# zju3dv/pvnet

Hardware: AMD Instinct MI355X
Metric: RANSAC votings/s (480x640, 9 kpts, batch 32) + HBM GB/s vs roofline (higher is better)
Workload: dtype f32 decisions (bf16x3 MFMA products, f32 accumulate; pairs inside the f32 rounding band re-evaluated in the reference's f32 order); refinement f64; 1 GPU; BASELINE.json configs[2]: batch=32 synthetic 480x640 fields per GPU, 9 keypoints, 1024 hypotheses, inlier_thresh 0.99, int64 mask, planar strided field; batch_per_gpu=32, global_batch=32, h=480, w=640, vn=9, hn=1024, mask_radius=40, field=noisy (0.05 rad + 10% outliers), N(0,1) background, input_sets_cycled=4, streams=6

## Files before the change

### include/pvnet_vote.h

```cpp
#ifndef PVNET_VOTE_H_
#define PVNET_VOTE_H_

#include <stddef.h>
#include <stdint.h>

#ifdef __cplusplus
extern "C" {
#endif

#define PVNET_VOTE_ABI_VERSION 9

#define PVNET_E_BADARG      (-1)
#define PVNET_E_WORKSPACE   (-2)
#define PVNET_E_UNSUPPORTED (-3)

#define PVNET_MASK_U8   0
#define PVNET_MASK_I16  1
#define PVNET_MASK_I32  2
#define PVNET_MASK_I64  3
#define PVNET_MASK_F32  4
#define PVNET_MASK_LOGITS_F32 5

#define PVNET_F_LITERAL   1u
#define PVNET_F_NO_REFINE 2u
// ... 87 lines not shown
                           float* out_kpts, int32_t* out_status,
                           void* workspace, size_t workspace_bytes, void* stream, float* stage_ms);

int pvnet_vote_v3_stage_repeat(const void* mask, int mask_dtype, const int64_t mask_strides[3],
                               const float* vertex, const int64_t vertex_strides[5],
                               int b, int h, int w, int vn, int hn,
                               float inlier_thresh, int min_num, int max_num,
                               uint64_t seed, int image_base, const int32_t* idxs, uint32_t flags,
                               float* out_kpts, int32_t* out_status,
                               void* workspace, size_t workspace_bytes, void* stream,
                               int stage, int repeats, float* avg_ms);

int pvnet_vote_band_margin(float thresh, uint32_t* out_stats, int b, int h, int w, int vn, int hn, int max_num,
                           void* workspace, size_t workspace_bytes, void* stream);

int pvnet_rccl_load(const char* path);
int pvnet_rccl_unique_id(void* id128);
int pvnet_rccl_comm_init(void** comm, int nranks, const void* id128, int rank);
int pvnet_rccl_comm_ranks(void* comm, int* nranks);
int pvnet_rccl_comm_destroy(void* comm);
int pvnet_vote_allgather(const float* local, float* all, size_t count_per_rank, void* comm, void* stream);

int pvnet_vote_confidence(const float* kpts, float thresh, float* out_conf, uint32_t vote_flags, int b, int h, int w,
                          int vn, int hn, int max_num, void* workspace, size_t workspace_bytes, void* stream);
int pvnet_vote_distribution(const float* mean, float* out_cov, int b, int h, int w, int vn, int hn, int max_num,
                            void* workspace, size_t workspace_bytes, void* stream);

size_t pvnet_motion_workspace_bytes(int b, int h, int w, int vn);
int pvnet_motion_voting(const void* mask, int mask_dtype, const int64_t mask_strides[3], const float* vertex,
                        const int64_t vertex_strides[5], int b, int h, int w, int vn, float* out_pts, void* workspace,
// ... 43 lines not shown
```

### pvnet_amd/_abi.py

```python
from __future__ import annotations

import ctypes as C
import functools
import os
from typing import NamedTuple

_HERE = os.path.dirname(os.path.abspath(__file__))
LIB_PATH = os.path.join(_HERE, "libpvnet_vote.so")
DEV_LIB_PATH = os.path.join(_HERE, "libpvnet_vote_dev.so")
TUNING_KNOBS = ("PVNET_SCORE_MODE", "PVNET_SCORE_WGS_PER_CU", "PVNET_SCORE_HPL", "PVNET_SCORE_CHUNK", "PVNET_COMPACT_KG",
                "PVNET_SCORE_XCD", "PVNET_SCORE_ATOMIC", "PVNET_SCORE_LDS_KB", "PVNET_SCORE_ACC", "PVNET_EXACT_FOLD",
                "PVNET_SCORE_RUNS", "PVNET_SCORE_CULL", "PVNET_CULL_Q_MILLI", "PVNET_DEV_STAGES")

ABI_VERSION = 9
E_BADARG, E_WORKSPACE, E_UNSUPPORTED = -1, -2, -3
MASK_U8, MASK_I16, MASK_I32, MASK_I64, MASK_F32, MASK_LOGITS_F32 = 0, 1, 2, 3, 4, 5
F_LITERAL = 1
F_NO_REFINE = 2
F_VERTEX_F16, F_VERTEX_BF16, F_LOGITS_F16, F_LOGITS_BF16 = 4, 8, 16, 32
F_APPROX = 64
F_BAND_STATS = 128
F_CONCURRENT = 256
F_CULL_ALL, F_CULL_NONE = 512, 1024
S_SKIPPED, S_SINGULAR, S_NO_INLIER, S_OVERFLOW = 1, 2, 4, 8
# ... 20 lines not shown
_WS_TAIL = [_int] * 6 + [_ptr, _size, _ptr]
_OP_GENERATE = [_ptr, _ptr, _ptr, _ptr, _int, _int, _int, _ptr]
_OP_VOTE = [_ptr, _ptr, _ptr, _ptr, _int, _int, _int, _f32, _ptr]
PROTOTYPES = {
    "pvnet_vote_abi_version": (_int, []),
    "pvnet_vote_build_info": (C.c_char_p, []),
    "pvnet_vote_tuning_reload": (None, []),
    "pvnet_vote_layout": (_int, [_int] * 6 + [C.POINTER(Layout)]),
    "pvnet_vote_workspace_bytes": (_size, [_int] * 6),
    "pvnet_vote_v3": (_int, _V3),
    "pvnet_vote_v3_logits": (_int, [_ptr, _i64p, _int, _ptr, _i64p] + _V3[5:]),
    "pvnet_vote_v3_prepared": (_int, _V3[3:6] + [_int] + _V3[6:]),
    "pvnet_vote_v3_profiled": (_int, _V3 + [C.POINTER(_f32)]),
    "pvnet_vote_v3_stage_repeat": (_int, _V3 + [_int, _int, C.POINTER(_f32)]),
    "pvnet_vote_band_margin": (_int, [_f32, _ptr] + _WS_TAIL),
    "pvnet_vote_confidence": (_int, [_ptr, _f32, _ptr, C.c_uint32] + _WS_TAIL),
    "pvnet_vote_distribution": (_int, [_ptr, _ptr] + _WS_TAIL),
    "pvnet_motion_workspace_bytes": (_size, [_int] * 4),
    "pvnet_motion_voting": (_int, [_ptr, _int, _i64p, _ptr, _i64p] + [_int] * 4 + [_ptr, _ptr, _size, _ptr]),
    "pvnet_motion_voting_typed": (_int, [_ptr, _int, _i64p, _ptr, _i64p] + [_int] * 4 + [C.c_uint32, _ptr, _ptr, _size, _ptr]),
    "pvnet_generate_hypothesis": (_int, _OP_GENERATE),
    "pvnet_voting_for_hypothesis": (_int, _OP_VOTE),
    "pvnet_generate_hypothesis_vanishing_point": (_int, _OP_GENERATE),
    "pvnet_voting_for_hypothesis_vanishing_point": (_int, _OP_VOTE),
    "pvnet_pose_solve": (_int, [_ptr, _int, _i64p, _ptr, _ptr, _int, _ptr] + [_int] * 4 + [_ptr] * 4),
    "pvnet_pose_metrics_workspace_bytes": (_size, [_int] * 3),
    "pvnet_pose_metrics": (_int, [_ptr, _ptr, _int] + [_ptr] * 4 + [_int, _int, _ptr, _ptr, _int, _int, _int, C.POINTER(C.c_double)] +
                           [_ptr] * 4 + [_size, _ptr]),
    "pvnet_nearest_workspace_bytes": (_size, [_int, _int]),
    "pvnet_nearest_point_idx": (_int, [_ptr, _ptr, _ptr] + [_int] * 5 + [_ptr, _size, _ptr]),
# ... 334 lines not shown
```

### pvnet_amd/csrc/epilogues.hip

```cpp
#include "vote_common.h"

namespace pvd {
namespace {

__global__ __launch_bounds__(256) void band_margin_kernel(VoteParams P, unsigned* __restrict__ out) {
    PVNET_SPARE_VGPRS(119);
    extern __shared__ __attribute__((aligned(16))) char smem[];
    uint4* s_t = reinterpret_cast<uint4*>(smem);
    float4* s_raw = reinterpret_cast<float4*>(s_t + 8 * TILE_U4);
    const int k = blockIdx.x % P.vn, bi = blockIdx.x / P.vn, grp = blockIdx.y;
    const int lane = threadIdx.x & 63, col = lane & 31, half = lane >> 5, wave = threadIdx.x >> 6;
    const int tn = P.ctrl[bi * CTRL_STRIDE + C_TN];
    if (P.ctrl[bi * CTRL_STRIDE + C_NCHUNKS] <= 0 || grp * 256 >= tn) return;
    const size_t bk = (size_t)bi * P.vn + k;
    const int tpad = (tn + PAD - 1) / PAD * PAD;
    const int32_t* const org = band_origin_ptr(P, bk);
    const float ox = (float)org[0], oy = (float)org[1];
    const float rho = band_rho(tn);
    {
        const int i = threadIdx.x, p = grp * 256 + i;
        float4 q = make_float4(0.f, 0.f, 0.f, 0.f);
        if (p < tpad) q = P.rec[bk * P.cap + p];
        s_raw[i] = q;
        uint4 r0, r1, r2, r3;
// ... 33 lines not shown
                if (!(fabsf(x) >= BAND_CLEAN)) ++nband;
                if ((x > 0.f) != lit) {
                    ++ndis;
                    worst = fmaxf(worst, fabsf(x));
                }
            }
        }
    }
    unsigned* o = out + bk * 4;
    if (worst > 0.f) atomicMax(o, __float_as_uint(worst));
    if (ndis) atomicAdd(o + 1, ndis);
    if (nband) atomicAdd(o + 2, nband);
    atomicAdd(o + 3, ntest);
}

__global__ __launch_bounds__(256) void ts_collect_kernel(const unsigned long long* __restrict__ stamps, int n,
                                                         unsigned long long* __restrict__ acc, int clear) {
    PVNET_SPARE_VGPRS(39);
    unsigned long long lo = ~0ull, hi = 0ull;
    for (int i = threadIdx.x; i < n; i += 256) {
        const unsigned long long a = stamps[2 * i], b = stamps[2 * i + 1];
        lo = a < lo ? a : lo;
        hi = b > hi ? b : hi;
    }
    __shared__ unsigned long long s_lo[256], s_hi[256];
    s_lo[threadIdx.x] = lo;
    s_hi[threadIdx.x] = hi;
    __syncthreads();
    if (threadIdx.x == 0) {
        for (int i = 1; i < 256; ++i) {
// ... 298 lines not shown
    if (!out_stats) return PVNET_E_BADARG;
    VoteParams P;
    int rc = params_for_workspace(P, b, h, w, vn, hn, max_num, workspace, workspace_bytes);
    if (rc) return rc;
    if (!(thresh >= 1e-3f && thresh < 1.f) || !P.mode) return PVNET_E_UNSUPPORTED;
    P.thresh = thresh;
    P.tau = (float)(sqrt(1.0 - (double)thresh * thresh) / (double)thresh);
    P.kband = band_constant(thresh);
    hipStream_t s = static_cast<hipStream_t>(stream);
    PV_HIP(hipMemsetAsync(out_stats, 0, sizeof(uint32_t) * 4 * (size_t)b * vn, s));
    const size_t lds = 8 * TILE_U4 * sizeof(uint4) + 256 * sizeof(float4);
    hipLaunchKernelGGL(band_margin_kernel, dim3((unsigned)(b * vn), (unsigned)((P.cap + 255) / 256)), dim3(256), lds, s, P,
                       reinterpret_cast<unsigned*>(out_stats));
    PV_LAUNCH_CHECK();
    return 0;
}

static int motion_layout(int b, int h, int w, int vn, size_t off[4], int* words, int* nseg) {
    if (b <= 0 || h <= 0 || w <= 0 || vn <= 0) return PVNET_E_BADARG;
    if ((long long)h * w > (1ll << 30) || b > 65535 || vn > 65535) return PVNET_E_UNSUPPORTED;
    *words = (int)(((long long)h * w + 63) / 64);
    *nseg = (*words + SEG_WORDS - 1) / SEG_WORDS;
    off[0] = 0;
    off[1] = align_up(off[0] + sizeof(uint64_t) * (size_t)b * *words, 256);
    off[2] = align_up(off[1] + sizeof(int32_t) * 2 * (size_t)b * *nseg, 256);
    off[3] = align_up(off[2] + sizeof(double) * 2 * (size_t)b * *nseg * vn, 256);
    return 0;
}

size_t pvnet_motion_workspace_bytes(int b, int h, int w, int vn) {
// ... 102 lines not shown
```

### pvnet_amd/csrc/k4_exact_body.h

```cpp
#pragma once
#include "vote_common.h"

namespace pvd {
namespace {

__device__ __forceinline__ void vote8x(unsigned& acc, float& dm, float a0, float b0, float a1, float b1, float a2, float b2,
                                       float a3, float b3, float a4, float b4, float a5, float b5, float a6, float b6,
                                       float a7, float b7) {
    float x0, x1, x2, x3;
    unsigned w0, w1;
    asm volatile(
        "v_sub_f32_e64 %2, %8, |%9|\n"
        "v_sub_f32_e64 %3, %10, |%11|\n"
        "v_sub_f32_e64 %4, %12, |%13|\n"
        "v_sub_f32_e64 %5, %14, |%15|\n"
        "v_min3_f32 %1, %1, |%2|, |%3|\n"
        "v_cvt_pknorm_u16_f32 %6, %2, %3\n"
        "v_sub_f32_e64 %2, %16, |%17|\n"
        "v_sub_f32_e64 %3, %18, |%19|\n"
        "v_min3_f32 %1, %1, |%4|, |%5|\n"
        "v_cvt_pknorm_u16_f32 %7, %4, %5\n"
        "v_sub_f32_e64 %4, %20, |%21|\n"
        "v_sub_f32_e64 %5, %22, |%23|\n"
        "v_add3_u32 %0, %6, %7, %0\n"
// ... 377 lines not shown
            for (int t = 0; t < MH; ++t) {
                flg[t] = dmn[t] >= BAND_CLEAN ? 0u : 1u;
                cnt[t] = flg[t] ? 0u : cnt[t];
            }
        }
        if (!RUNS) flush_counts<MH>(P.counts + it.bk * P.hn_pad + it.h0, cnt);
        list_flagged_cells<MH>(P, flg, it.h0, lane, wave, colx, halfx, s_cells, &s_ncell);
        lds_barrier();
        clk.mark(2);
        const int ncell = s_ncell;
        if (ncell > 0) {
            int tid2 = threadIdx.x;
            asm volatile("" : "+v"(tid2));
            const int grp = tid2 >> 4, q = tid2 & 15;
            int ntests = 0;
            for (int e = grp; e < ncell; e += 16) {
                const unsigned cell = s_cells[e];
                const int hl = (int)(cell & 1023u), hf = (int)((cell >> 10) & 1u);
                unsigned m = cell >> 11;
                const float2 hv = s_hyp[hl];
                const int row = (q >> 2) * 8 + hf * 4 + (q & 3);
                int votes = 0;
                while (m) {
                    const int g = __ffs((int)m) - 1;
                    m &= m - 1u;
                    const int t0 = FOLD ? nti - 1 - g : 0, t1 = FOLD ? t0 + 1 : nti;
                    for (int tile = t0; tile < t1; ++tile) {
                        const float4 r = s_raw[tile * 32 + row];
                        votes += inlier_literal(r.x, r.y, r.z, r.w, hv.x, hv.y, P.thresh) ? 1 : 0;
                        ++ntests;
                    }
                }
                add_cell_votes(P.counts + it.bk * P.hn_pad + it.hslice + hl, votes, q);
            }
            add_band_stats(P, tid2, q, ncell, ntests);
        }
    }
    if (RUNS && run_key >= 0) flush_counts<MH>(P.counts + run_bk * P.hn_pad + run_h0, cnt);
    if (!HEAD) clk.finish(P);
}
#undef PV_XS
#undef PV_LO
#undef PV_HI

}
// ... 2 lines not shown
```

### pvnet_amd/csrc/k4_score_cull.hip

```cpp
#include "vote_common.h"
#include "k4_exact_body.h"

namespace pvd {
namespace {

template <bool TIMED, bool TAIL, bool WIDE>
__device__ __forceinline__ void score_cull_body(VoteParams P) {
    constexpr int MH = 8;
    if (WIDE) PVNET_SPARE_VGPRS(135); else PVNET_SPARE_VGPRS(127);
    if (!TAIL) PhaseClock<TIMED>::stamp(P, 0);
    extern __shared__ __attribute__((aligned(16))) char smem[];
    int tx0 = threadIdx.x;
    if (TAIL) asm volatile("" : "+v"(tx0));
    const int lane = tx0 & 63, col = lane & 31, half = lane >> 5;
    const int wave = __builtin_amdgcn_readfirstlane((int)(threadIdx.x >> 6));
    uint4* s_t = reinterpret_cast<uint4*>(smem);
    unsigned* s_cells = reinterpret_cast<unsigned*>(s_t + 9 * TILE_U4);
    uint8_t* s_list = reinterpret_cast<uint8_t*>(s_cells + 4 * MH * 64);
    float* s_sig = reinterpret_cast<float*>(s_list + 32 * CULL_NPX);
    int* s_nu = reinterpret_cast<int*>(s_sig + CULL_NPX);
    int* s_cv = s_nu + 32;
    __shared__ int s_ncell;
    const int32_t* __restrict__ ctrl = P.ctrl;
    const int total = ctrl[P.b * CTRL_STRIDE];
// ... 185 lines not shown
            }
        }
        clk.mark(2);
        int lx = lane;
        asm volatile("" : "+v"(lx));
        const int colx = lx & 31, halfx = lx >> 5;
        flush_counts<MH>(P.cnts + it.bk * P.hn_pad + it.h0, cnt);
        list_flagged_cells<MH>(P, flg, it.h0, lane, wave, colx, halfx, s_cells, &s_ncell);
        lds_barrier();
        const int ncell = s_ncell;
        if (ncell > 0) {
            int tid2 = threadIdx.x;
            asm volatile("" : "+v"(tid2));
            const int grp = tid2 >> 4, q = tid2 & 15;
            int ntests = 0;
            for (int e = grp; e < ncell; e += 16) {
                const unsigned cell = s_cells[e];
                const int hl = (int)(cell & 1023u), hf = (int)((cell >> 10) & 1u);
                unsigned m = cell >> 11;
                const float2 hv = P.hyps[it.bk * P.hn_pad + it.hslice + hl];
                const int j = hl >> 5;
                const int nu = s_nu[j], ng = (nu + 31) >> 5;
                const int row = (q >> 2) * 8 + hf * 4 + (q & 3);
                int votes = 0;
                while (m) {
                    const int gb = __ffs((int)m) - 1;
                    m &= m - 1u;
                    const int slot = (ng - 1 - gb) * 32 + row;
                    if (slot < nu) {
                        const int px = it.cg * CULL_NPX + (int)s_list[j * CULL_NPX + slot];
                        const float4 r = P.rec[it.bk * P.cap + px];
                        votes += inlier_literal(r.x, r.y, r.z, r.w, hv.x, hv.y, P.thresh) ? 1 : 0;
                        ++ntests;
                    }
                }
                add_cell_votes(P.cnts + it.bk * P.hn_pad + it.hslice + hl, votes, q);
            }
            add_band_stats(P, tid2, q, ncell, ntests);
        }
    }
    if ((P.flags & PVNET_F_BAND_STATS) && lane == 0) {
        atomicAdd(P.ctrl + P.b * CTRL_STRIDE + 1, (int)st_steps);
        atomicAdd(P.ctrl + P.b * CTRL_STRIDE + 7, (int)st_full);
    }
    clk.finish(P);
}
#define PV_DEF_SCORE_BOTH(TIMED_, RUNS_, NVGPR_)                                                                          \
    __global__ __launch_bounds__(256) __attribute__((amdgpu_waves_per_eu(3, 8), amdgpu_num_vgpr(NVGPR_ / 2))) void        \
// ... 31 lines not shown
```

### pvnet_amd/csrc/k5_refine.hip

```cpp
#include "vote_common.h"

namespace pvd {
namespace {

constexpr int RT = PVNET_RT;
constexpr int RW = RT / 64;
template <bool LITERAL>
__global__ __launch_bounds__(RT) void select_refine_kernel(VoteParams P) {
    PVNET_SPARE_VGPRS(71);
    small_stage_prio();
    const int k = blockIdx.x, bi = blockIdx.y;
    const int wave = threadIdx.x >> 6, lane = threadIdx.x & 63;
    const size_t bk = (size_t)bi * P.vn + k;
    const int nchunks = P.ctrl[bi * CTRL_STRIDE + C_NCHUNKS];
    const int nch = (!LITERAL && P.mode) ? (nchunks + P.wg_s - 1) / P.wg_s : nchunks;
    int status = P.ctrl[bi * CTRL_STRIDE + C_STATUS];

    __shared__ unsigned long long s_best[RW];
    __shared__ double s_sum[RW][5];
    __shared__ int s_n[RW];

    if (nch == 0) {
        if (threadIdx.x < 2) P.out[bk * 2 + threadIdx.x] = 0.f;
        if (threadIdx.x == 0) {
            if (P.status) P.status[bk] = status | PVNET_S_SKIPPED;
            P.win[bk * 2] = 0;
            P.win[bk * 2 + 1] = 0;
        }
        for (int h = threadIdx.x; h < P.hn; h += RT) P.counts[bk * P.hn_pad + h] = 0;
        return;
    }
    unsigned long long best = 0;
    const size_t row = (size_t)(P.hn_pad >> 1);
    if (!LITERAL && P.cull && *kp_cull_ptr(P, bk) != 0) {
        for (int p = threadIdx.x; p < P.hn_pad; p += RT) {
// ... 55 lines not shown
        P.win[bk * 2] = widx;
        P.win[bk * 2 + 1] = wcnt;
    }
    if (P.flags & PVNET_F_NO_REFINE) {
        if (threadIdx.x == 0) {
            P.out[bk * 2] = wx;
            P.out[bk * 2 + 1] = wy;
            if (P.status) P.status[bk] = status;
        }
        return;
    }
    const int tn = P.ctrl[bi * CTRL_STRIDE + C_TN];
    const float ox = (float)P.ctrl[bi * CTRL_STRIDE + C_OX], oy = (float)P.ctrl[bi * CTRL_STRIDE + C_OY];
    double a = 0, bb = 0, d = 0, r0 = 0, r1 = 0;
    int n = 0;
#pragma unroll 4
    for (int t = threadIdx.x; t < tn; t += RT) {
        const float4 q = P.rec[bk * P.cap + t];
        const float2 u = rec_dir(q);
        bool in;
        if (LITERAL || P.exact) {
            in = inlier_literal(q.x, q.y, u.x, u.y, wx, wy, P.thresh);
        } else {
            float4 ra;
            float2 rb;
            make_pixrec(q, P.tau, ox, oy, ra, rb);
            in = vote_expanded(ra, rb, wx - ox, wy - oy) > 0.5f;
        }
        const double nx = in ? (double)u.y : 0.0, ny = in ? -(double)u.x : 0.0;
        const double bv = nx * ((double)q.x - (double)wx) + ny * ((double)q.y - (double)wy);
        a += nx * nx;
        bb += nx * ny;
        d += ny * ny;
        r0 += nx * bv;
        r1 += ny * bv;
        n += in ? 1 : 0;
    }
    a = wave_reduce_add(a);
    bb = wave_reduce_add(bb);
    d = wave_reduce_add(d);
    r0 = wave_reduce_add(r0);
    r1 = wave_reduce_add(r1);
    n = wave_reduce_add(n);
    if (lane == 0) {
        s_sum[wave][0] = a; s_sum[wave][1] = bb; s_sum[wave][2] = d; s_sum[wave][3] = r0; s_sum[wave][4] = r1;
        s_n[wave] = n;
    }
    __syncthreads();
    if (threadIdx.x == 0) {
        a = bb = d = r0 = r1 = 0;
        n = 0;
        for (int i = 0; i < RW; ++i) {
            a += s_sum[i][0]; bb += s_sum[i][1]; d += s_sum[i][2]; r0 += s_sum[i][3]; r1 += s_sum[i][4];
            n += s_n[i];
        }
        const double det = a * d - bb * bb;
        float rx = wx, ry = wy;
        if (n == 0 || det == 0.0 || !isfinite(det)) {
            status |= PVNET_S_SINGULAR;
        } else {
            rx = (float)((double)wx + (d * r0 - bb * r1) / det);
            ry = (float)((double)wy + (a * r1 - bb * r0) / det);
        }
// ... 18 lines not shown
```

### pvnet_amd/csrc/vote_common.h

```cpp
#pragma once
#include <hip/hip_runtime.h>

#include <math.h>
#include <stdint.h>
#include <stdlib.h>

#include "pvnet_rng.h"
#include "pvnet_vote.h"

namespace pvd {

__device__ constexpr float kF1e6 = 0x1.0c6f7ap-20f;

constexpr int CTRL_STRIDE = 8;
enum { C_TN0 = 0, C_TN = 1, C_STATUS = 2, C_ITEM_BASE = 3, C_NCHUNKS = 4, C_OX = 5, C_OY = 6,
       C_RHO = 7 };

constexpr int SEG_WORDS = 64;
#ifndef PVNET_K1_WAVES
#define PVNET_K1_WAVES 8
#endif
#ifndef PVNET_RT
#define PVNET_RT 512
#endif
// ... 51 lines not shown
    float2* hyp;
    uint4* hypb;
    uint16_t* partial;
    int32_t* counts;
    int32_t* win;
    float* out;
    int32_t* status;
    int cull;
    float cull_q;
    int32_t* perm;
    float2* hyps;
    int32_t* cnts;
    uint4* hypc;
    float* hypg;
    int src_div;
};

constexpr int CF_ANY_CULLED = 0;
constexpr int CF_VOTES_NOW = 1, CF_BATCH_OK = 2;
__device__ __forceinline__ int32_t* call_flags_ptr(const VoteParams& P) {
    return P.ctrl + (size_t)(P.b + 1) * CTRL_STRIDE + 3 * (size_t)P.b * P.vn;
}


__device__ __forceinline__ void hyp_intersect(float ux0, float uy0, float cx0, float cy0, float ux1, float uy1,
                                              float cx1, float cy1, float& ox, float& oy) {
#pragma clang fp contract(off)
    const float nx0 = uy0, ny0 = -ux0, nx1 = uy1, ny1 = -ux1;
    const float dety = nx1 * ny0 - nx0 * ny1;
    const float detx = ny1 * nx0 - ny0 * nx1;
    ox = 0.f;
    oy = 0.f;
    if (fabsf(dety) <= kF1e6 || fabsf(detx) <= kF1e6) return;
    const float b0 = nx0 * cx0 + ny0 * cy0;
    const float b1 = nx1 * cx1 + ny1 * cy1;
    oy = (nx1 * b0 - nx0 * b1) / dety;
    ox = (ny1 * b0 - ny0 * b1) / detx;
}

__device__ __forceinline__ bool inlier_literal(float cx, float cy, float nx, float ny, float hx, float hy,
                                               float thresh) {
#pragma clang fp contract(off)
    const float dx = hx - cx, dy = hy - cy;
    const float norm1 = __builtin_sqrtf(nx * nx + ny * ny);
    const float norm2 = __builtin_sqrtf(dx * dx + dy * dy);
    if (norm1 <= kF1e6 || norm2 <= kF1e6) return false;
    const float ang = (dx * nx + dy * ny) / (norm1 * norm2);
    return ang > thresh;
}

__device__ __forceinline__ float norm1_literal(float nx, float ny) {
#pragma clang fp contract(off)
    return __builtin_sqrtf(nx * nx + ny * ny);
}

__device__ __forceinline__ float2 rec_dir(float4 q) { return make_float2(q.z, q.w); }
__device__ __forceinline__ float vote_scale(float ux, float uy) {
    const float m = fmaxf(fabsf(ux), fabsf(uy));
    const uint32_t e = (__float_as_uint(m) >> 23) & 0xFFu;
    uint32_t f = 314u - e;
    f = f > 254u ? 254u : f;
    return __uint_as_float(f << 23);
}
__device__ __forceinline__ void make_pixrec(float4 q, float tau, float ox, float oy, float4& a, float2& b) {
    const float cx = q.x - ox, cy = q.y - oy;
    const float sc = vote_scale(q.z, q.w);
    const float My = q.w * sc, nMx = -q.z * sc;
    const float2 tq = make_float2(tau * -nMx, tau * My);
// ... 167 lines not shown
__device__ __forceinline__ int item_kp(int y) { return y & 0xFFFF; }
__device__ __forceinline__ bool item_culled(int y) { return (y >> ITEM_CULL_SHIFT) != 0; }

constexpr int CULL_NPX = 256;
constexpr int CULL_HN = 1024;
constexpr int CULL_DEAD = 8 * TILE_U4_;
constexpr int NCAND = 8, KP_MAX = 32;

__device__ __forceinline__ int32_t* kp_cull_ptr(const VoteParams& P, size_t bk) {
    return P.ctrl + (size_t)(P.b + 1) * CTRL_STRIDE + 2 * (size_t)P.b * P.vn + bk;
}

constexpr int OR_READY = 0, OR_VOTE = 1;
__device__ __forceinline__ int32_t* origin_ready_ptr(const VoteParams& P, int bi) {
    return P.ctrl + (size_t)(P.b + 1) * CTRL_STRIDE + 3 * (size_t)P.b * P.vn + 8 + 2 * (size_t)bi;
}

struct KpShared {
    float cand[KP_MAX * NCAND * 2];
    float med[KP_MAX * 2];
    int org[KP_MAX * 2];
    int vote[KP_MAX];
};
__device__ __forceinline__ bool image_culled(const KpShared& S, int vn) {
    int votes = 0;
    for (int kk = 0; kk < vn; ++kk) votes += S.vote[kk];
    return 2 * votes > vn;
}
__device__ __forceinline__ void kp_origin_vote(const VoteParams& P, int tn, bool live, int pm, bool mine, const float4& q0, const float4& q1,
                                               KpShared& S) {
// ... 100 lines not shown
    int chunk;
    int compact_kg;
    int score_xcd;
    int score_lds_kb;
    int score_atomic;
    int score_acc;
    int score_runs;
    int score_cull;
    int cull_q_milli;
    int exact_fold;
    int dev_stages;
    int cus;
};
Tuning& tuning();
void load_tuning(Tuning& t);
float band_constant(float thresh);
int layout_fingerprint(const PvnetVoteLayout& L);
int fill_params(VoteParams& P, const void* mask, int mask_dtype, const int64_t* ms, const float* vertex, const int64_t* vs, int b,
                int h, int w, int vn, int hn, float thresh, int min_num, int max_num, uint64_t seed, int image_base,
                const int32_t* idxs, uint32_t flags, float* out, int32_t* status, void* ws, size_t ws_bytes);

#define PV_LAUNCH_CHECK()                                   \
    do {                                                    \
        hipError_t e_ = hipGetLastError();                  \
        if (e_ != hipSuccess) return (int)e_;               \
    } while (0)
#define PV_HIP(x)                                           \
    do {                                                    \
        hipError_t e_ = (x);                                \
        if (e_ != hipSuccess) return (int)e_;               \
    } while (0)
// ... 13 lines not shown
```

### pvnet_amd/csrc/vote_host.hip

```cpp
#include "vote_common.h"

namespace pvd {

float band_constant(float thresh) {
    const double u = ldexp(1.0, -24), t = (double)thresh;
    const double tau = sqrt(1.0 - t * t) / t, t0 = acos(t), delta = 10.0 * u;
    const double lo = acos(t + delta < 1.0 ? t + delta : 1.0), hi = acos(t - delta);
    const double k_side = sin(t0 - lo) > sin(hi - t0) ? sin(t0 - lo) : sin(hi - t0);
    const double k_lit = k_side / t * 1.001;
    const double k_fast = u * (1.0 + tau) * (1.43 * 10.0 + 8.0);
    return (float)(k_lit + k_fast);
}
int band_fold1(int forced) {
    return forced == 0 ? 0 : 1;
}

constexpr uint64_t CTRL_BLOCK_REVISION = 2;
int layout_fingerprint(const PvnetVoteLayout& L) {
    uint64_t x = 0x9E3779B97F4A7C15ull;
    const uint64_t v[] = {CTRL_BLOCK_REVISION, (uint64_t)L.chunk, (uint64_t)L.hpl, (uint64_t)L.wg_g, (uint64_t)L.reserved_, (uint64_t)L.cap,
                          (uint64_t)L.hn_pad, (uint64_t)L.off_rec, (uint64_t)L.off_hyp, (uint64_t)L.off_counts,
                          (uint64_t)L.off_win, (uint64_t)L.total_bytes, (uint64_t)L.cull, (uint64_t)L.off_perm, (uint64_t)L.off_hypc};
    for (uint64_t e : v) { x ^= e + 0x9E3779B97F4A7C15ull + (x << 6) + (x >> 2); }
    const int fp = (int)(x ^ (x >> 32));
    return fp ? fp : 1;
}

#ifdef PVNET_DEV
int env_int(const char* name, int dflt) {
    const char* s = getenv(name);
    return (s && *s) ? atoi(s) : dflt;
}
// ... 129 lines not shown
    if ((flags & PVNET_F_VERTEX_F16) && (flags & PVNET_F_VERTEX_BF16)) return PVNET_E_BADARG;
    if ((flags & PVNET_F_LOGITS_F16) && (flags & PVNET_F_LOGITS_BF16)) return PVNET_E_BADARG;
    P.vertex_type = (flags & PVNET_F_VERTEX_F16) ? VT_F16 : (flags & PVNET_F_VERTEX_BF16) ? VT_BF16 : VT_F32;
    P.logits_type = (flags & PVNET_F_LOGITS_F16) ? VT_F16 : (flags & PVNET_F_LOGITS_BF16) ? VT_BF16 : VT_F32;
    P.b = b; P.h = h; P.w = w; P.vn = vn; P.hn = hn; P.npix = h * w;
    P.words = L.words; P.cap = L.cap; P.chunk = L.chunk; P.max_chunks = L.max_chunks;
    P.hpl = L.hpl; P.hgroups = L.hgroups; P.hn_pad = L.hn_pad; P.wg_g = L.wg_g; P.wg_s = L.wg_s;
    P.mode = L.reserved_;
    P.layout_fp = layout_fingerprint(L);
    P.score_xcd = tuning().score_xcd;
    P.atomic_counts = tuning().score_atomic;
    P.thresh = thresh;
    P.tau = (thresh > 0.f && thresh < 1.f) ? (float)(sqrt(1.0 - (double)thresh * thresh) / (double)thresh) : 0.f;
    if (!(flags & (PVNET_F_LITERAL | PVNET_F_APPROX)) && !L.reserved_) flags |= PVNET_F_LITERAL;
    P.exact = (!(flags & (PVNET_F_LITERAL | PVNET_F_APPROX)) && L.reserved_) ? 1 : 0;
    P.kband = P.exact ? band_constant(thresh) : 0.f;
    P.fold1 = P.exact ? band_fold1(tuning().exact_fold) : 0;
    if (P.exact && P.fold1 && (L.wg_s * L.chunk) / 32 > 21) P.fold1 = 0;
    if (P.exact) P.atomic_counts = 1;
    P.min_num = min_num; P.max_num = max_num; P.seed = seed; P.image_base = image_base; P.idxs = idxs; P.flags = flags;
    P.ctrl = reinterpret_cast<int32_t*>(base + L.off_ctrl);
    P.items = reinterpret_cast<int4*>(base + L.off_items);
    P.seg = reinterpret_cast<int32_t*>(base + L.off_seg);
    P.seg0 = P.seg + (size_t)L.b * L.nseg;
    P.cum = max_num < h * (long long)w
                ? reinterpret_cast<uint16_t*>(base + L.off_seg + align_up(sizeof(int32_t) * 2 * (size_t)L.b * L.nseg, 16))
                : nullptr;
    P.nseg = L.nseg;
    P.bits = reinterpret_cast<uint64_t*>(base + L.off_bits);
    P.pix = reinterpret_cast<int32_t*>(base + L.off_pix);
    P.rec = reinterpret_cast<float4*>(base + L.off_rec);
// ... 71 lines not shown
    if (mode && (4 / wg_g) * chunk / 2 >= VOTE_WRAP) return PVNET_E_UNSUPPORTED;
    L->b = b; L->h = h; L->w = w; L->vn = vn; L->hn = hn;
    L->cap = (int)cap;
    L->words = (int)((npix + 63) / 64);
    L->chunk = chunk;
    L->max_chunks = (int)((cap + chunk - 1) / chunk);
    L->hpl = hpl;
    L->hgroups = hgroups;
    L->hn_pad = hgroups * 64 * hpl;
    L->wg_g = wg_g;
    L->wg_s = 4 / wg_g;
    L->reserved_ = mode ? 1 : 0;
    size_t off = 0;
    auto take = [&](size_t bytes) { size_t o = off; off = align_up(off + bytes, 256); return o; };
    L->nseg = (L->words + SEG_WORDS - 1) / SEG_WORDS;
    L->off_ctrl = take(sizeof(int32_t) * (CTRL_STRIDE * (size_t)(b + 1) + 3 * (size_t)b * vn + 8 + 2 * (size_t)b));
    L->off_seg = take(align_up(sizeof(int32_t) * 2 * (size_t)b * L->nseg, 16) +
                      (max_num < npix ? sizeof(uint16_t) * THIN_BINS * (size_t)b * L->nseg : 0));
    L->off_items = take(sizeof(int32_t) * 4 * (size_t)b * vn * (hgroups / wg_g) *
                        (size_t)((L->max_chunks + L->wg_s - 1) / L->wg_s));
    L->off_bits = take(sizeof(uint64_t) * (size_t)b * L->words);
    L->off_pix = take(sizeof(int32_t) * (size_t)b * cap);
    L->off_rec = take(sizeof(float) * 4 * (size_t)b * vn * cap);
    L->off_hyp = take(sizeof(float) * 2 * (size_t)b * vn * L->hn_pad);
    L->off_hypb = take(mode ? sizeof(uint4) * 2 * (size_t)b * vn * L->hn_pad : 0);
    L->off_partial = take(T.score_atomic ? 0 : sizeof(uint16_t) * (size_t)b * vn * L->max_chunks * L->hn_pad);
    L->off_counts = take(sizeof(int32_t) * (size_t)b * vn * L->hn_pad);
    L->off_win = take(sizeof(int32_t) * 2 * (size_t)b * vn);
    L->cull = (cull_knob && mode && T.score_atomic && wg_g * hpl / 2 == 8 && L->wg_s * chunk == CULL_NPX && L->hn_pad == CULL_HN && vn <= KP_MAX) ? 1 : 0;
    L->off_perm = take(L->cull ? sizeof(int32_t) * (size_t)b * vn * L->hn_pad : 0);
    L->off_hyps = take(L->cull ? sizeof(float) * 2 * (size_t)b * vn * L->hn_pad : 0);
// ... 133 lines not shown
```

### pvnet_amd/voting.py

```python
from __future__ import annotations

import ctypes as C
import struct
from typing import Optional

import torch

from ._abi import (CLASSES_MAX, DEV_LIB_PATH, LIB_PATH, TUNING_KNOBS, Layout, _check, _wanted_library, load_classes_library,
                   load_library, reload_tuning, vote_layout)
from ._abi import (F_APPROX, F_BAND_STATS, F_CONCURRENT, F_CULL_ALL, F_CULL_NONE, F_LITERAL, F_LOGITS_BF16,
                   F_LOGITS_F16, F_NO_REFINE, F_VERTEX_BF16, F_VERTEX_F16, MASK_F32, MASK_I16, MASK_I32, MASK_I64, MASK_U8,
                   NUM_STAGES, S_NO_INLIER, S_OVERFLOW, S_SINGULAR, S_SKIPPED, STAGE_NAMES)
from ._marshal import strides as _strides

_FIELD_FLAGS = {torch.float32: 0, torch.float16: F_VERTEX_F16, torch.bfloat16: F_VERTEX_BF16}
_LOGITS_FLAGS = {torch.float32: 0, torch.float16: F_LOGITS_F16, torch.bfloat16: F_LOGITS_BF16}
_MASK_CODES = {torch.uint8: MASK_U8, torch.int8: MASK_U8, torch.bool: MASK_U8, torch.int16: MASK_I16, torch.int32: MASK_I32,
               torch.int64: MASK_I64, torch.float32: MASK_F32}


def _clamp_max_num(max_num) -> int:
    return int(min(max(int(max_num), 0), 2 ** 31 - 1))


# ... 72 lines not shown
    cull = {}
    if L.cull:
        cull = dict(perm=view(L.off_perm, 4 * b * vn * hp, torch.int32, (b, vn, hp)),
                    hyps=view(L.off_hyps, 8 * b * vn * hp, torch.float32, (b, vn, hp, 2)))
    return _DebugViews(
        **cull,
        layout=L, ctrl=ctrl, tn0=ctrl[:b, 0], tn=ctrl[:b, 1], nchunks=ctrl[:b, 4], total_items=ctrl[b, 0],
        bits=view(L.off_bits, 8 * b * L.words, torch.int64, (b, L.words)),
        pix=view(L.off_pix, 4 * b * cap, torch.int32, (b, cap)),
        rec=view(L.off_rec, 16 * b * vn * cap, torch.float32, (b, vn, cap, 4)),
        hyp=view(L.off_hyp, 8 * b * vn * hp, torch.float32, (b, vn, hp, 2))[:, :, :L.hn],
        counts=view(L.off_counts, 4 * b * vn * hp, torch.int32, (b, vn, hp))[:, :, :L.hn],
        win=view(L.off_win, 8 * b * vn, torch.int32, (b, vn, 2)),
        band_origin=view(L.off_ctrl + 4 * 8 * (b + 1), 8 * b * vn, torch.int32, (b, vn, 2)),
        cull_bits=view(L.off_ctrl + 4 * 8 * (b + 1) + 8 * b * vn, 4 * b * vn, torch.int32, (b, vn)),
    )


def effective_literal(literal: bool, inlier_thresh: float) -> bool:
    t = float(inlier_thresh)
    t32 = struct.unpack('f', struct.pack('f', t))[0]
    return bool(literal) or not (struct.unpack('f', struct.pack('f', 1e-3))[0] <= t32 < 1.0)


def mode_flags(literal: bool, approx: bool, inlier_thresh: float) -> int:
    if effective_literal(literal, inlier_thresh):
        return F_LITERAL
    return F_APPROX if approx else _CULL_FLAG


# ... 75 lines not shown
            _check(lib.pvnet_vote_v3(*args), "pvnet_vote_v3")
    extras = []
    if return_status:
        extras.append(status)
    if return_debug:
        d = _debug_views(ws, L)
        d["literal"] = bool(literal)
        d["mode"] = "literal" if (literal or (not approx and not L.reserved_)) else ("approx" if approx else "exact")
        d["concurrent"] = bool(flags & F_CONCURRENT)
        if not (d["mode"] == "exact" and L.cull):
            d["cull"] = False
            d["cull_bits"] = torch.zeros((b, vn), dtype=torch.int32, device=dev)
        if band_stats:
            d["band_stats"] = tuple(int(x) for x in d["ctrl"][b, 4:6].tolist())
            d["cull_stats"] = (int(d["ctrl"][b, 1]), int(d["ctrl"][b, 7]))
        d["status"] = status
        d["seed"] = seed
        d["workspace"] = ws
        d["max_num"] = max_num
        extras.append(d)
    if stage_times:
        extras.append(times)
    return (out, *extras) if extras else out


def band_margin(dbg, inlier_thresh):
    L, ws = dbg["layout"], dbg["workspace"]
    dev = ws.device
    out = torch.zeros((L.b * L.vn, 4), dtype=torch.int32, device=dev)
    with torch.cuda.device(dev):
# ... 446 lines not shown
```

Baseline: 237,900 votings/s.

## Use certified fast inlier test in refine, bare sqrt in literal path

The refine kernel in exact mode now classifies each pixel with a cheap cross/dot margin test and falls back to the literal sqrt/divide test only when some lane in the wave lands inside a rounding-uncertain band. The loop is also restructured to batch four record loads before evaluating them. The literal test swaps the library sqrt for a hardware sqrt plus a one-ulp correction meant to give the correctly rounded result. Test counting in the scoring kernels is now gated behind the stats flag. A debug probe kernel and refine stats buffer are added; the risks are correctness of the clear-band constant and extra control-block workspace.

Result: no change. 240,000 votings/s, median of 6 (+0.9%).

```diff
diff --git a/include/pvnet_vote.h b/include/pvnet_vote.h
--- a/include/pvnet_vote.h
+++ b/include/pvnet_vote.h
@@ -125,6 +125,8 @@
 int pvnet_vote_band_margin(float thresh, uint32_t* out_stats, int b, int h, int w, int vn, int hn, int max_num,
                            void* workspace, size_t workspace_bytes, void* stream);
 
+int pvnet_vote_literal_probe(int mode, const float* rows, int64_t n, uint32_t* out, void* stream);
+
 int pvnet_rccl_load(const char* path);
 int pvnet_rccl_unique_id(void* id128);
 int pvnet_rccl_comm_init(void** comm, int nranks, const void* id128, int rank);
diff --git a/pvnet_amd/_abi.py b/pvnet_amd/_abi.py
--- a/pvnet_amd/_abi.py
+++ b/pvnet_amd/_abi.py
@@ -58,6 +58,7 @@
     "pvnet_vote_v3_profiled": (_int, _V3 + [C.POINTER(_f32)]),
     "pvnet_vote_v3_stage_repeat": (_int, _V3 + [_int, _int, C.POINTER(_f32)]),
     "pvnet_vote_band_margin": (_int, [_f32, _ptr] + _WS_TAIL),
+    "pvnet_vote_literal_probe": (_int, [_int, _ptr, C.c_int64, _ptr, _ptr]),
     "pvnet_vote_confidence": (_int, [_ptr, _f32, _ptr, C.c_uint32] + _WS_TAIL),
     "pvnet_vote_distribution": (_int, [_ptr, _ptr] + _WS_TAIL),
     "pvnet_motion_workspace_bytes": (_size, [_int] * 4),
diff --git a/pvnet_amd/csrc/epilogues.hip b/pvnet_amd/csrc/epilogues.hip
--- a/pvnet_amd/csrc/epilogues.hip
+++ b/pvnet_amd/csrc/epilogues.hip
@@ -71,6 +71,52 @@
     atomicAdd(o + 3, ntest);
 }
 
+#ifdef PVNET_DEV
+__device__ __forceinline__ bool inlier_literal_builtin_sqrt(float cx, float cy, float nx, float ny, float hx, float hy, float thresh) {
+#pragma clang fp contract(off)
+    const float dx = hx - cx, dy = hy - cy;
+    const float norm1 = __builtin_sqrtf(nx * nx + ny * ny);
+    const float norm2 = __builtin_sqrtf(dx * dx + dy * dy);
+    if (norm1 <= kF1e6 || norm2 <= kF1e6) return false;
+    const float ang = (dx * nx + dy * ny) / (norm1 * norm2);
+    return ang > thresh;
+}
+__global__ __launch_bounds__(256) void sqrt_bare_sweep_kernel(unsigned* __restrict__ out) {
+    PVNET_SPARE_VGPRS(31);
+    const unsigned T = gridDim.x * 256u, i0 = blockIdx.x * 256u + threadIdx.x;
+    int ngate = 0, nval = 0;
+    for (unsigned long long p = i0; p < (1ull << 32); p += T) {
+        const unsigned bits = (unsigned)p;
+        const bool nan = (bits & 0x7FFFFFFFu) > 0x7F800000u;
+        if ((bits >> 31) && !nan) continue;
+        const float a = __uint_as_float(bits);
+        const float r0 = __builtin_sqrtf(a), r1 = sqrt_rn_bare(a);
+        const bool g0 = r0 <= kF1e6, g1 = r1 <= kF1e6;
+        ngate += g0 != g1 ? 1 : 0;
+        nval += (!g0 && !g1 && __float_as_uint(r0) != __float_as_uint(r1)) ? 1 : 0;
+    }
+    ngate = wave_reduce_add(ngate);
+    nval = wave_reduce_add(nval);
+    __shared__ int s_n[4][2];
+    if ((threadIdx.x & 63) == 0) { s_n[threadIdx.x >> 6][0] = ngate; s_n[threadIdx.x >> 6][1] = nval; }
+    __syncthreads();
+    if (threadIdx.x < 2) {
+        const int v = (s_n[0][threadIdx.x] + s_n[1][threadIdx.x]) + (s_n[2][threadIdx.x] + s_n[3][threadIdx.x]);
+        if (v) atomicAdd(out + threadIdx.x, (unsigned)v);
+    }
+}
+__global__ __launch_bounds__(256) void literal_rows_kernel(const float* __restrict__ rows, long long n, unsigned* __restrict__ out) {
+    PVNET_SPARE_VGPRS(31);
+    const long long i = (long long)blockIdx.x * 256 + threadIdx.x;
+    if (i >= n) return;
+    const float* r = rows + i * 7;
+    const bool a = inlier_literal(r[0], r[1], r[2], r[3], r[4], r[5], r[6]);
+    const bool b = inlier_literal_builtin_sqrt(r[0], r[1], r[2], r[3], r[4], r[5], r[6]);
+    out[i] = (a ? 1u : 0u) | (b ? 2u : 0u);
+}
+
+#endif
+
 __global__ __launch_bounds__(256) void ts_collect_kernel(const unsigned long long* __restrict__ stamps, int n,
                                                          unsigned long long* __restrict__ acc, int clear) {
     PVNET_SPARE_VGPRS(39);
@@ -399,6 +445,26 @@
                        reinterpret_cast<unsigned*>(out_stats));
     PV_LAUNCH_CHECK();
     return 0;
+}
+
+int pvnet_vote_literal_probe(int mode, const float* rows, int64_t n, uint32_t* out, void* stream) {
+    if (!out || (mode != 0 && mode != 1)) return PVNET_E_BADARG;
+    if (mode == 1 && (!rows || n <= 0 || n > (int64_t)1 << 30)) return PVNET_E_BADARG;
+#ifdef PVNET_DEV
+    hipStream_t s = static_cast<hipStream_t>(stream);
+    if (mode == 0) {
+        PV_HIP(hipMemsetAsync(out, 0, sizeof(uint32_t) * 2, s));
+        hipLaunchKernelGGL(sqrt_bare_sweep_kernel, dim3(4096), dim3(256), 0, s, reinterpret_cast<unsigned*>(out));
+    } else {
+        hipLaunchKernelGGL(literal_rows_kernel, dim3((unsigned)((n + 255) / 256)), dim3(256), 0, s, rows, (long long)n,
+                           reinterpret_cast<unsigned*>(out));
+    }
+    PV_LAUNCH_CHECK();
+    return 0;
+#else
+    (void)stream;
+    return PVNET_E_UNSUPPORTED;
+#endif
 }
 
 static int motion_layout(int b, int h, int w, int vn, size_t off[4], int* words, int* nseg) {
diff --git a/pvnet_amd/csrc/k4_exact_body.h b/pvnet_amd/csrc/k4_exact_body.h
--- a/pvnet_amd/csrc/k4_exact_body.h
+++ b/pvnet_amd/csrc/k4_exact_body.h
@@ -415,10 +415,12 @@
             asm volatile("" : "+v"(tid2));
             const int grp = tid2 >> 4, q = tid2 & 15;
             int ntests = 0;
+            const bool stats = (P.flags & PVNET_F_BAND_STATS) != 0;
             for (int e = grp; e < ncell; e += 16) {
                 const unsigned cell = s_cells[e];
                 const int hl = (int)(cell & 1023u), hf = (int)((cell >> 10) & 1u);
                 unsigned m = cell >> 11;
+                if (stats) ntests += __popc(m) * (FOLD ? 1 : nti);
                 const float2 hv = s_hyp[hl];
                 const int row = (q >> 2) * 8 + hf * 4 + (q & 3);
                 int votes = 0;
@@ -429,7 +431,6 @@
                     for (int tile = t0; tile < t1; ++tile) {
                         const float4 r = s_raw[tile * 32 + row];
                         votes += inlier_literal(r.x, r.y, r.z, r.w, hv.x, hv.y, P.thresh) ? 1 : 0;
-                        ++ntests;
                     }
                 }
                 add_cell_votes(P.counts + it.bk * P.hn_pad + it.hslice + hl, votes, q);
diff --git a/pvnet_amd/csrc/k4_score_cull.hip b/pvnet_amd/csrc/k4_score_cull.hip
--- a/pvnet_amd/csrc/k4_score_cull.hip
+++ b/pvnet_amd/csrc/k4_score_cull.hip
@@ -223,6 +223,7 @@
             asm volatile("" : "+v"(tid2));
             const int grp = tid2 >> 4, q = tid2 & 15;
             int ntests = 0;
+            const bool stats = (P.flags & PVNET_F_BAND_STATS) != 0;
             for (int e = grp; e < ncell; e += 16) {
                 const unsigned cell = s_cells[e];
                 const int hl = (int)(cell & 1023u), hf = (int)((cell >> 10) & 1u);
@@ -240,7 +241,7 @@
                         const int px = it.cg * CULL_NPX + (int)s_list[j * CULL_NPX + slot];
                         const float4 r = P.rec[it.bk * P.cap + px];
                         votes += inlier_literal(r.x, r.y, r.z, r.w, hv.x, hv.y, P.thresh) ? 1 : 0;
-                        ++ntests;
+                        if (stats) ++ntests;
                     }
                 }
                 add_cell_votes(P.cnts + it.bk * P.hn_pad + it.hslice + hl, votes, q);
diff --git a/pvnet_amd/csrc/k5_refine.hip b/pvnet_amd/csrc/k5_refine.hip
--- a/pvnet_amd/csrc/k5_refine.hip
+++ b/pvnet_amd/csrc/k5_refine.hip
@@ -19,6 +19,9 @@
     __shared__ unsigned long long s_best[RW];
     __shared__ double s_sum[RW][5];
     __shared__ int s_n[RW];
+    __shared__ int s_st[RW][2];
+    const bool stats = !LITERAL && P.exact && (P.flags & PVNET_F_BAND_STATS);
+    if (stats && threadIdx.x < 2) refine_stats_ptr(P, bk)[threadIdx.x] = 0;
 
     if (nch == 0) {
         if (threadIdx.x < 2) P.out[bk * 2 + threadIdx.x] = 0.f;
@@ -104,13 +107,30 @@
     const float ox = (float)P.ctrl[bi * CTRL_STRIDE + C_OX], oy = (float)P.ctrl[bi * CTRL_STRIDE + C_OY];
     double a = 0, bb = 0, d = 0, r0 = 0, r1 = 0;
     int n = 0;
-#pragma unroll 4
-    for (int t = threadIdx.x; t < tn; t += RT) {
-        const float4 q = P.rec[bk * P.cap + t];
+    int st_lit = 0, st_cert = 0;
+    auto take = [&](const float4 q) __attribute__((always_inline)) {
         const float2 u = rec_dir(q);
         bool in;
-        if (LITERAL || P.exact) {
+        if (LITERAL) {
             in = inlier_literal(q.x, q.y, u.x, u.y, wx, wy, P.thresh);
+        } else if (P.exact) {
+            const float dx = wx - q.x, dy = wy - q.y;
+            const float dot = fmaf(dx, u.x, dy * u.y), crs = fmaf(dx, u.y, -(dy * u.x));
+            const float m = fmaf(P.tau, dot, -fabsf(crs));
+            const float dd = fmaf(dx, dx, dy * dy), uu = fmaf(u.x, u.x, u.y * u.y);
+            const float S = dd * uu;
+            const bool clear = m * m > P.kclear2 * S && fminf(dd, uu) >= 0x1p-38f && S <= 0x1p120f;
+            in = m > 0.f;
+            const unsigned long long unclear = __ballot(!clear);
+            if (unclear) {
+                float qx = q.x;
+                asm volatile("" : "+v"(qx));
+                in = inlier_literal(qx, q.y, u.x, u.y, wx, wy, P.thresh);
+            }
+            if (stats) {
+                if (unclear) ++st_lit;
+                else st_cert += (int)__popcll(__ballot(true));
+            }
         } else {
             float4 ra;
             float2 rb;
@@ -125,6 +145,26 @@
         r0 += nx * bv;
         r1 += ny * bv;
         n += in ? 1 : 0;
+    };
+    const float4* const rec = P.rec + bk * P.cap;
+    int t0 = 0;
+    for (; t0 + 4 * RT <= tn; t0 += 4 * RT) {
+        float4 qs[4];
+#pragma unroll
+        for (int j = 0; j < 4; ++j) qs[j] = rec[t0 + j * RT + (int)threadIdx.x];
+#pragma unroll
+        for (int j = 0; j < 4; ++j) take(qs[j]);
+    }
+    {
+        float4 qs[4];
+#pragma unroll
+        for (int j = 0; j < 4; ++j) {
+            const int t = t0 + j * RT + (int)threadIdx.x;
+            if (t0 + j * RT < tn) qs[j] = rec[t < tn ? t : tn - 1];
+        }
+#pragma unroll
+        for (int j = 0; j < 4; ++j)
+            if (t0 + j * RT + (int)threadIdx.x < tn) take(qs[j]);
     }
     a = wave_reduce_add(a);
     bb = wave_reduce_add(bb);
@@ -135,8 +175,14 @@
     if (lane == 0) {
         s_sum[wave][0] = a; s_sum[wave][1] = bb; s_sum[wave][2] = d; s_sum[wave][3] = r0; s_sum[wave][4] = r1;
         s_n[wave] = n;
+        if (stats) { s_st[wave][0] = st_lit; s_st[wave][1] = st_cert; }
     }
     __syncthreads();
+    if (stats && threadIdx.x < 2) {
+        int v = 0;
+        for (int i = 0; i < RW; ++i) v += s_st[i][threadIdx.x];
+        refine_stats_ptr(P, bk)[threadIdx.x] = v;
+    }
     if (threadIdx.x == 0) {
         a = bb = d = r0 = r1 = 0;
         n = 0;
diff --git a/pvnet_amd/csrc/vote_common.h b/pvnet_amd/csrc/vote_common.h
--- a/pvnet_amd/csrc/vote_common.h
+++ b/pvnet_amd/csrc/vote_common.h
@@ -89,6 +89,8 @@
     uint4* hypc;
     float* hypg;
     int src_div;
+    float kband_lit;
+    float kclear2;
 };
 
 constexpr int CF_ANY_CULLED = 0;
@@ -113,12 +115,20 @@
     ox = (ny1 * b0 - ny0 * b1) / detx;
 }
 
+__device__ __forceinline__ float sqrt_rn_bare(float a) {
+    const float s = __builtin_amdgcn_sqrtf(a);
+    const float sm = __uint_as_float(__float_as_uint(s) - 1u), sp = __uint_as_float(__float_as_uint(s) + 1u);
+    const float rm = __builtin_fmaf(-sm, s, a), rp = __builtin_fmaf(-sp, s, a);
+    const float t = rm <= 0.f ? sm : s;
+    return rp > 0.f ? sp : t;
+}
+
 __device__ __forceinline__ bool inlier_literal(float cx, float cy, float nx, float ny, float hx, float hy,
                                                float thresh) {
 #pragma clang fp contract(off)
     const float dx = hx - cx, dy = hy - cy;
-    const float norm1 = __builtin_sqrtf(nx * nx + ny * ny);
-    const float norm2 = __builtin_sqrtf(dx * dx + dy * dy);
+    const float norm1 = sqrt_rn_bare(nx * nx + ny * ny);
+    const float norm2 = sqrt_rn_bare(dx * dx + dy * dy);
     if (norm1 <= kF1e6 || norm2 <= kF1e6) return false;
     const float ang = (dx * nx + dy * ny) / (norm1 * norm2);
     return ang > thresh;
@@ -126,7 +136,7 @@
 
 __device__ __forceinline__ float norm1_literal(float nx, float ny) {
 #pragma clang fp contract(off)
-    return __builtin_sqrtf(nx * nx + ny * ny);
+    return sqrt_rn_bare(nx * nx + ny * ny);
 }
 
 __device__ __forceinline__ float2 rec_dir(float4 q) { return make_float2(q.z, q.w); }
@@ -324,6 +334,10 @@
 constexpr int OR_READY = 0, OR_VOTE = 1;
 __device__ __forceinline__ int32_t* origin_ready_ptr(const VoteParams& P, int bi) {
     return P.ctrl + (size_t)(P.b + 1) * CTRL_STRIDE + 3 * (size_t)P.b * P.vn + 8 + 2 * (size_t)bi;
+}
+
+__device__ __forceinline__ int32_t* refine_stats_ptr(const VoteParams& P, size_t bk) {
+    return P.ctrl + (size_t)(P.b + 1) * CTRL_STRIDE + 3 * (size_t)P.b * P.vn + 8 + 2 * (size_t)P.b + 2 * bk;
 }
 
 struct KpShared {
@@ -454,7 +468,8 @@
 };
 Tuning& tuning();
 void load_tuning(Tuning& t);
-float band_constant(float thresh);
+float band_constant(float thresh, float* k_lit = nullptr);
+float refine_clear_constant2(float thresh, float k_lit);
 int layout_fingerprint(const PvnetVoteLayout& L);
 int fill_params(VoteParams& P, const void* mask, int mask_dtype, const int64_t* ms, const float* vertex, const int64_t* vs, int b,
                 int h, int w, int vn, int hn, float thresh, int min_num, int max_num, uint64_t seed, int image_base,
diff --git a/pvnet_amd/csrc/vote_host.hip b/pvnet_amd/csrc/vote_host.hip
--- a/pvnet_amd/csrc/vote_host.hip
+++ b/pvnet_amd/csrc/vote_host.hip
@@ -2,20 +2,27 @@
 
 namespace pvd {
 
-float band_constant(float thresh) {
+float band_constant(float thresh, float* k_lit_out) {
     const double u = ldexp(1.0, -24), t = (double)thresh;
     const double tau = sqrt(1.0 - t * t) / t, t0 = acos(t), delta = 10.0 * u;
     const double lo = acos(t + delta < 1.0 ? t + delta : 1.0), hi = acos(t - delta);
     const double k_side = sin(t0 - lo) > sin(hi - t0) ? sin(t0 - lo) : sin(hi - t0);
     const double k_lit = k_side / t * 1.001;
     const double k_fast = u * (1.0 + tau) * (1.43 * 10.0 + 8.0);
+    if (k_lit_out) *k_lit_out = (float)k_lit;
     return (float)(k_lit + k_fast);
+}
+float refine_clear_constant2(float thresh, float k_lit) {
+    const double u = ldexp(1.0, -24), t = (double)thresh;
+    const double tau = sqrt(1.0 - t * t) / t;
+    const double kappa = ((double)k_lit + 5.0 * u * (1.0 + tau)) * 1.001;
+    return nextafterf((float)(kappa * kappa), INFINITY);
 }
 int band_fold1(int forced) {
     return forced == 0 ? 0 : 1;
 }
 
-constexpr uint64_t CTRL_BLOCK_REVISION = 2;
+constexpr uint64_t CTRL_BLOCK_REVISION = 3;
 int layout_fingerprint(const PvnetVoteLayout& L) {
     uint64_t x = 0x9E3779B97F4A7C15ull;
     const uint64_t v[] = {CTRL_BLOCK_REVISION, (uint64_t)L.chunk, (uint64_t)L.hpl, (uint64_t)L.wg_g, (uint64_t)L.reserved_, (uint64_t)L.cap,
@@ -175,7 +182,9 @@
     P.tau = (thresh > 0.f && thresh < 1.f) ? (float)(sqrt(1.0 - (double)thresh * thresh) / (double)thresh) : 0.f;
     if (!(flags & (PVNET_F_LITERAL | PVNET_F_APPROX)) && !L.reserved_) flags |= PVNET_F_LITERAL;
     P.exact = (!(flags & (PVNET_F_LITERAL | PVNET_F_APPROX)) && L.reserved_) ? 1 : 0;
-    P.kband = P.exact ? band_constant(thresh) : 0.f;
+    P.kband_lit = 0.f;
+    P.kband = P.exact ? band_constant(thresh, &P.kband_lit) : 0.f;
+    P.kclear2 = P.exact ? refine_clear_constant2(thresh, P.kband_lit) : 0.f;
     P.fold1 = P.exact ? band_fold1(tuning().exact_fold) : 0;
     if (P.exact && P.fold1 && (L.wg_s * L.chunk) / 32 > 21) P.fold1 = 0;
     if (P.exact) P.atomic_counts = 1;
@@ -277,7 +286,7 @@
     size_t off = 0;
     auto take = [&](size_t bytes) { size_t o = off; off = align_up(off + bytes, 256); return o; };
     L->nseg = (L->words + SEG_WORDS - 1) / SEG_WORDS;
-    L->off_ctrl = take(sizeof(int32_t) * (CTRL_STRIDE * (size_t)(b + 1) + 3 * (size_t)b * vn + 8 + 2 * (size_t)b));
+    L->off_ctrl = take(sizeof(int32_t) * (CTRL_STRIDE * (size_t)(b + 1) + 3 * (size_t)b * vn + 8 + 2 * (size_t)b + 2 * (size_t)b * vn));
     L->off_seg = take(align_up(sizeof(int32_t) * 2 * (size_t)b * L->nseg, 16) +
                       (max_num < npix ? sizeof(uint16_t) * THIN_BINS * (size_t)b * L->nseg : 0));
     L->off_items = take(sizeof(int32_t) * 4 * (size_t)b * vn * (hgroups / wg_g) *
diff --git a/pvnet_amd/voting.py b/pvnet_amd/voting.py
--- a/pvnet_amd/voting.py
+++ b/pvnet_amd/voting.py
@@ -110,6 +110,7 @@
         win=view(L.off_win, 8 * b * vn, torch.int32, (b, vn, 2)),
         band_origin=view(L.off_ctrl + 4 * 8 * (b + 1), 8 * b * vn, torch.int32, (b, vn, 2)),
         cull_bits=view(L.off_ctrl + 4 * 8 * (b + 1) + 8 * b * vn, 4 * b * vn, torch.int32, (b, vn)),
+        refine_stats=view(L.off_ctrl + 4 * (8 * (b + 1) + 3 * b * vn + 8 + 2 * b), 8 * b * vn, torch.int32, (b, vn, 2)),
     )
 
 
@@ -215,6 +216,8 @@
         if band_stats:
             d["band_stats"] = tuple(int(x) for x in d["ctrl"][b, 4:6].tolist())
             d["cull_stats"] = (int(d["ctrl"][b, 1]), int(d["ctrl"][b, 7]))
+        if not (band_stats and d["mode"] == "exact"):
+            del d["refine_stats"]
         d["status"] = status
         d["seed"] = seed
         d["workspace"] = ws
```
